# benedikthoward/ENPH459-Super-Resolution

Measured on AMD Instinct MI355X. Metric: HR megapixels/sec at x4 upscale (SAA + 80-iteration IBP reconstruction), higher is better.
Workload: dtype f32; 1 GPU; C2: x4 multi-frame SR of 64x64 LR patches -> 256x256 HR, N=16 frames (all 4x4 sub-pixel phases), 7x7 Gaussian PSF, shift_and_add + ibp(80 it, step 0.5); patches_per_gpu=1024, global_patches=1024, factor=4, frames=16, n_iter=80, parallelism=patch-sharded x1, no collective

## Files before the change

### enph459-super-resolution_amd/csrc/srx_patch.hpp

```cpp
#pragma once
#include "srx_mosaic.hpp"

namespace srx {
namespace patch {

#ifndef SRX_PARK16
#define SRX_PARK16 1
#endif
#ifndef SRX_ADDTID
#define SRX_ADDTID 1
#endif
#ifndef SRX_M0_NOP
#define SRX_M0_NOP "s_nop 0\n\t"
#endif
#ifndef SRX_TRANSPOSE_DEF
#define SRX_TRANSPOSE_DEF 1
#endif
#ifndef SRX_PATCH_DBG
#define SRX_PATCH_DBG 0
#endif
constexpr int PN = 256;
constexpr int TSD = 68;
constexpr int RW = 32 * TSD;
constexpr int SLOT0 = 0, SLOT1 = 1024;
constexpr int FIX = 16;
constexpr int YW = 260;
constexpr int OFF_YT = 16 * RW, OFF_YL = OFF_YT + 4 * YW, OFF_GT = OFF_YL + 4 * YW, OFF_GL = OFF_GT + 3 * YW,
              OFF_ROW = OFF_GL + 3 * YW, OFF_PART = OFF_ROW + PN, LDS_WORDS = OFF_PART + 32;
static_assert(LDS_WORDS * 4 <= 160 * 1024, "LDS budget");

constexpr double ZD = -0.26794919243112270647;
constexpr float PZ = (float)ZD;
constexpr float K2 = (float)(1.0 / (1.0 - ZD));
constexpr float K1 = (float)(1.0 / ((1.0 - ZD) * (1.0 - ZD)));
constexpr float K3 = (float)(ZD / (1.0 - ZD * ZD));
constexpr float K4 = (float)(1.0 / (1.0 - ZD * ZD));
struct ZPow {
    float v[FIX];
    constexpr ZPow() : v()
    {
        double p = ZD;
        for (int i = 0; i < FIX; i++) {
            v[i] = (float)p;
            p *= ZD;
        }
    }
};
__device__ constexpr ZPow ZP{};

typedef float f8 __attribute__((ext_vector_type(8)));
struct AxisW {
    float kb[8];
    float kt[8];
    float wfb[8];
};
struct AxisC {
    int ex;
    int nb;
    int E;
};
__device__ __forceinline__ f8 sload8(const float *p)
{
    f8 v;
    asm volatile("s_load_dwordx8 %0, %1, 0x0\n\ts_waitcnt lgkmcnt(0)" : "=s"(v) : "s"(p) : "memory");
    return v;
}

constexpr int NN_PAD = 2048;

struct PatchArgs {
    AxisC y, x;
    int nn, ntop;
    int ngrp;
    int c01;
    unsigned long long ry[4], rx[4];
    float sn;
};

struct PatchTabs {
    const float *Mt;
    const unsigned *Mt8;
    const int *m8;
    const float *Ct;
    const AxisW *aw;
    const uint2 *nrec;
    const uint2 *nent;
    const float2 *Mn;
    const float *k2;
};

static inline bool axis_ok(const mosaic::AxisPlan &pl, int f)
{
    const int nmin = pl.nmin, nmax = pl.nmax;
    return !pl.zero && nmax >= 0 && nmax <= 1 && nmin <= 0 && nmax - nmin <= 3 && nmax - nmin <= f - 1 && -nmin < f;
}

static inline bool shape_admits(int elem_bytes, int H, int W) { return elem_bytes == 4 && H == PN && W == PN; }

static inline bool eligible(int elem_bytes, int N, int H, int W, const double *sh, const double *k, int kh, int kw, int f, bool rank1_only = false)
{
    if (!shape_admits(elem_bytes, H, W) || f < 2)
        return false;
    mosaic::AxisPlan py, px;
    if (!mosaic::plan_axis(N, sh, 0, f, py) || !mosaic::plan_axis(N, sh, 1, f, px))
        return false;
    fused::Kernel7<float> kc;
    fused::make_kernel7<float>(k, kh, kw, false, kc);
    if (!((kc.separable || !rank1_only) && axis_ok(py, f) && axis_ok(px, f)))
        return false;
    const int exy = py.nmax, nby = -py.nmin, exx = px.nmax, nbx = -px.nmin;
    return (exy + nby) * (PN + exx) + (PN - nby) * (exx + nbx) <= NN_PAD;
}

__global__ void __launch_bounds__(256)
    k_patch_prep(const float *__restrict__ Mg, const float *__restrict__ Cg, int B, int Hg, int Wg, int nby, int nbx, float *__restrict__ Mt,
                 float *__restrict__ Ct, unsigned *__restrict__ Mt8, int *__restrict__ m8)
{
    __shared__ float t[32][33];
    const int b = blockIdx.z, x0 = blockIdx.x * 32, y0 = blockIdx.y * 32;
    const float *src = b < B ? Mg + (size_t)b * Hg * Wg : Cg;
    float *dst = b < B ? Mt + (size_t)b * PN * PN : Ct;
    bool ok = true;
    for (int r = threadIdx.y; r < 32; r += 8) {
        float v = src[(size_t)(y0 + r + 13) * Wg + x0 + threadIdx.x + 13];
        if (b < B && (y0 + r < nby || x0 + (int)threadIdx.x < nbx))
            v = 0.f;
        ok = ok && v == rintf(v) && v >= 0.f && v <= 255.f;
        t[r][threadIdx.x] = v;
    }
    __syncthreads();
    const int g = threadIdx.y;
    reinterpret_cast<float4 *>(dst)[(size_t)(x0 / 4 + g) * PN + y0 + threadIdx.x] =
        make_float4(t[threadIdx.x][4 * g], t[threadIdx.x][4 * g + 1], t[threadIdx.x][4 * g + 2], t[threadIdx.x][4 * g + 3]);
    if (b < B) {
        const unsigned w = (unsigned)t[threadIdx.x][4 * g] | (unsigned)t[threadIdx.x][4 * g + 1] << 8 |
                           (unsigned)t[threadIdx.x][4 * g + 2] << 16 | (unsigned)t[threadIdx.x][4 * g + 3] << 24;
        const int wr = x0 / 4 + g;
        Mt8[(size_t)b * (PN / 4) * PN + ((size_t)(wr >> 2) * PN + y0 + threadIdx.x) * 4 + (wr & 3)] = w;
    }
    const bool bad = __syncthreads_or(b < B && !ok);
    if (bad && threadIdx.x == 0 && threadIdx.y == 0)
        atomicAnd(&m8[b], 0);
}

__device__ __forceinline__ void near_coords(int t, int exy, int exx, int nby, int nbx, int &ngy, int &ngx, int &dst)
{
    const int WN = PN + exx, LN = exx + nbx, ntop = (exy + nby) * WN;
    if (t < ntop) {
        const int rr = t / WN, cc = t - rr * WN;
        ngy = rr - exy, ngx = cc - exx, dst = rr * YW + cc;
    } else {
        const int q = t - ntop, rr = q / LN, cc = q - rr * LN;
        ngy = nby + rr, ngx = cc - exx, dst = 3 * YW + rr * 3 + cc;
    }
}
__device__ __forceinline__ int strip_off(int ry, int rx, int exy, int exx, int nby)
{
    return ry <= nby ? (ry + exy) * YW + rx + exx : 4 * YW + (ry + exy) * 4 + rx + exx;
}

__global__ void __launch_bounds__(256)
    k_patch_near_tab(const int *__restrict__ ncu, const int *__restrict__ nyx, int NS, int PBy, int PBx, int exy, int exx, int nby,
                     int nbx, int Ey, int Ex, int nn, uint2 *__restrict__ nrec, uint2 *__restrict__ nent)
{
    const int t = blockIdx.x * 256 + threadIdx.x;
    if (t >= nn)
        return;
    int ngy, ngx, dst;
    near_coords(t, exy, exx, nby, nbx, ngy, ngx, dst);
    const int ni = mosaic::near_index(ngy + 13, ngx + 13, PN + 27, PBy, PBx), pk = ncu[ni], cnt = pk & 255, cu = pk >> 8;
    const int own = strip_off(ngy, ngx, exy, exx, nby);
    nrec[t] = make_uint2((unsigned)cnt | (unsigned)cu << 8 | (unsigned)dst << 16, (unsigned)own);
    for (int g = 0; g < NS / 4; g++) {
        unsigned o[4];
        for (int e = 0; e < 4; e++) {
            const int c = nyx[(size_t)ni * NS + 4 * g + e];
            o[e] = 4 * g + e < cnt ? (unsigned)strip_off((c & 0xffff) - Ey, (c >> 16) - Ex, exy, exx, nby) : (unsigned)own;
        }
        nent[(size_t)g * NN_PAD + t] = make_uint2(o[0] | o[1] << 16, o[2] | o[3] << 16);
    }
}

__global__ void __launch_bounds__(256)
    k_patch_near_m(const float *__restrict__ Mg, const float *__restrict__ Mu, int NB, int PBy, int PBx, int exy, int exx, int nby, int nbx,
                   int nn, float2 *__restrict__ Mn)
{
    const int t = blockIdx.x * 256 + threadIdx.x, b = blockIdx.y;
    if (t >= nn)
        return;
    int ngy, ngx, dst;
    near_coords(t, exy, exx, nby, nbx, ngy, ngx, dst);
    const int Wg = PN + 27, ni = mosaic::near_index(ngy + 13, ngx + 13, Wg, PBy, PBx);
    Mn[(size_t)b * NN_PAD + t] = make_float2(Mg[((size_t)b * Wg + ngy + 13) * Wg + ngx + 13], Mu[(size_t)b * NB + ni]);
}

struct AxisMap {
    signed char cls[PN];
    unsigned char idx[PN];
};
struct BuildMaps {
    AxisMap y, x;
    signed char frame[4][4];
    int nby, nbx;
};
__global__ void k_patch_maps(BuildMaps v, BuildMaps *dst)
{
    const int *s = reinterpret_cast<const int *>(&v);
    int *d = reinterpret_cast<int *>(dst);
    for (int i = threadIdx.x; i < (int)(sizeof(BuildMaps) / 4); i += blockDim.x)
        d[i] = s[i];
}
template <int PASS, typename S = float, bool WIDE = false>
__global__ void __launch_bounds__(256)
    k_patch_build(const S *__restrict__ lr, int N, int h, int w, const BuildMaps *__restrict__ maps, int *__restrict__ m8,
                  float *__restrict__ Mt, unsigned *__restrict__ Mt8)
{
    __shared__ float4 tile[64][17];
    const int b = blockIdx.y, gy0 = blockIdx.x * 16, cq = threadIdx.x & 63, wv = threadIdx.x >> 6;
    constexpr bool bytes = PASS == 0, test = PASS == 0 && std::is_same<S, float>::value;
    static_assert(PASS == 0 || std::is_same<S, float>::value, "byte frames need no float plane");
    if (PASS == 1 && __builtin_amdgcn_readfirstlane(m8[b]) != 0)
        return;
    int bad = 0;
    const S *src = lr + (size_t)b * N * h * w;
    int cx[4], jx[4];
#pragma unroll
    for (int c = 0; c < 4; c++) {
        const int gx = 4 * cq + c;
        cx[c] = gx < maps->nbx ? -1 : maps->x.cls[gx];
        jx[c] = maps->x.idx[gx];
    }
    const int *fw = reinterpret_cast<const int *>(&maps->frame[0][0]);
    const int fr0 = fw[0], fr1 = fw[1], fr2 = fw[2], fr3 = fw[3];
    float v[4][4];
    bool done = false;
    if constexpr (WIDE) {
        __shared__ unsigned rowsw[4][4][64];
        if ((((size_t)lr) & 3) == 0) {
            const int nd = w >> 2, kx = cq / nd, dw = cq - kx * nd;
            unsigned wd[4];
#pragma unroll
            for (int m = 0; m < 4; m++) {
                const int gy = gy0 + wv + 4 * m;
                const int cy = gy < maps->nby ? -1 : (int)maps->y.cls[gy], iy = maps->y.idx[gy];
                const int fsel = cy == 0 ? fr0 : cy == 1 ? fr1 : cy == 2 ? fr2 : fr3;
                wd[m] = 0;
                if (cy >= 0)
                    wd[m] = reinterpret_cast<const unsigned *>(src + ((size_t)((fsel >> (8 * kx)) & 0xff) * h + iy) * w)[dw];
            }
#pragma unroll
            for (int m = 0; m < 4; m++)
                rowsw[wv][m][cq] = wd[m];
            __syncthreads();
            const unsigned char *rb = reinterpret_cast<const unsigned char *>(&rowsw[wv][0][0]);
#pragma unroll
            for (int m = 0; m < 4; m++) {
                const int gy = gy0 + wv + 4 * m;
                const int cy = gy < maps->nby ? -1 : (int)maps->y.cls[gy];
#pragma unroll
                for (int c = 0; c < 4; c++) {
                    v[m][c] = 0.f;
                    if (cy >= 0 && cx[c] >= 0)
                        v[m][c] = (float)rb[m * 256 + cx[c] * w + jx[c]];
                }
            }
            done = true;
        }
    }
    if (!done)
#pragma unroll
    for (int m = 0; m < 4; m++) {
        const int gy = gy0 + wv + 4 * m;
        const int cy = gy < maps->nby ? -1 : (int)maps->y.cls[gy], iy = maps->y.idx[gy];
        const int fsel = cy == 0 ? fr0 : cy == 1 ? fr1 : cy == 2 ? fr2 : fr3;
#pragma unroll
        for (int c = 0; c < 4; c++) {
            v[m][c] = 0.f;
            if (cy >= 0 && cx[c] >= 0)
                v[m][c] = src[((size_t)((fsel >> (8 * cx[c])) & 0xff) * h + iy) * w + jx[c]];
        }
    }
#pragma unroll
    for (int m = 0; m < 4; m++) {
        if (test) {
#pragma unroll
            for (int c = 0; c < 4; c++)
                bad |= !((int)(v[m][c] == rintf(v[m][c])) & (int)(v[m][c] >= 0.f) & (int)(v[m][c] <= 255.f));
        }
        tile[cq][wv + 4 * m] = make_float4(v[m][0], v[m][1], v[m][2], v[m][3]);
    }
    if (test) {
        if (__syncthreads_or(bad) && threadIdx.x == 0)
            atomicAnd(&m8[b], 0);
    } else {
        __syncthreads();
    }
    if (bytes) {
#pragma unroll
        for (int n = 0; n < 4; n++) {
            const int u = threadIdx.x + 256 * n, sub = u & 3, r = (u >> 2) & 15, grp = u >> 6, q = 4 * grp + sub;
            const float4 t = tile[q][r];
            const unsigned wd = (unsigned)t.x | (unsigned)t.y << 8 | (unsigned)t.z << 16 | (unsigned)t.w << 24;
            Mt8[(size_t)b * (PN / 4) * PN + ((size_t)grp * PN + gy0 + r) * 4 + sub] = wd;
        }
    } else {
#pragma unroll
        for (int n = 0; n < 4; n++) {
            const int u = threadIdx.x + 256 * n, r = u & 15, q = u >> 4;
            reinterpret_cast<float4 *>(Mt)[((size_t)b * (PN / 4) + q) * PN + gy0 + r] = tile[q][r];
        }
// ... 178 lines not shown
        for (int i = 0; i < FIX; i++)
            a[i] = fmaf(ZP.v[i], carry, a[i]);
    }
    const float cb = last ? fmaf(a[63] - blast * K2, K3, blast * K1) : 0.f;
    chain64<true>(a, cb);
    float cm1 = 0.f, cm2 = 0.f;
    if (first) {
        const float qs = bfirst * K2;
        cm1 = fmaf(z, a[0], qs);
        cm2 = fmaf(z, cm1, qs);
        const float cm3 = fmaf(z, cm2, qs);
        yex = wfb[0] * cm3 + wfb[1] * cm2 + wfb[2] * cm1 + wfb[3] * a[0];
    }
    Rown[sb + lane] = a[0];
    Rown[sb + 64 + lane] = a[62];
    Rown[sb + 128 + lane] = a[63];
    __syncthreads();
    float hb = cb;
    if (!last) {
        hb = Rnext[sb + lane];
#pragma unroll
        for (int i = 0; i < FIX; i++)
            a[63 - i] = fmaf(ZP.v[i], hb, a[63 - i]);
    }
    if (!first) {
        cm2 = fmaf(ZP.v[1], a[0], Rprev[sb + 64 + lane]);
        cm1 = fmaf(ZP.v[0], a[0], Rprev[sb + 128 + lane]);
    }
    float c2 = cm2, c1 = cm1;
#pragma unroll
    for (int i = 0; i < 64; i++) {
        const float c0 = a[i], cn = i < 63 ? a[i + 1] : hb;
        a[i] = wfb[0] * c2 + wfb[1] * c1 + wfb[2] * c0 + wfb[3] * cn;
        c2 = c1, c1 = c0;
    }
}

template <bool BLUR, typename F, typename P>
__device__ __forceinline__ void bwd_chain_x(float (&a)[64], float (&out)[64], bool first, bool last, float *Rown, const float *Rprev,
                                            const float *Rnext, int s1, int s6, int lane, const f8 wfb, const f8 kt, float gm1, float gp1,
                                            float gp2, float gtop, F mid, P post, float (&hlo)[3], float (&hhi)[3])
{
    const float z = PZ;
    const float w0 = wfb[4], w1 = wfb[5], w2 = wfb[6], w3 = wfb[7];
    const float vn = last ? w0 * a[63] : 0.f;
    SRX_PSTAMP(15);
    float st = 0.f;
    if (first) {
        st = (w0 + w1 + w2 + w3) * gtop * K2;
        st = fmaf(z, st, (w0 + w1 + w2) * gtop + w3 * a[0]);
        st = fmaf(z, st, (w0 + w1) * gtop + w2 * a[0] + w3 * a[1]);
    }
    float gprev = gm1;
#pragma unroll
    for (int t = 0; t < 64; t++) {
        const float g0 = a[t], g1 = t < 63 ? a[t + 1] : gp1, g2 = t < 62 ? a[t + 2] : (t == 62 ? gp1 : gp2);
        a[t] = w0 * gprev + w1 * g0 + w2 * g1 + w3 * g2;
        gprev = g0;
    }
    chain64<false>(a, st);
    SRX_PSTAMP(16);
    Rown[s1 + lane] = a[63];
    __syncthreads();
    SRX_PSTAMP(17);
    if (!first) {
        const float carry = Rprev[s1 + lane];
#pragma unroll
        for (int i = 0; i < FIX; i++)
            a[i] = fmaf(ZP.v[i], carry, a[i]);
    }
    const float cb = last ? fmaf(z, a[63], vn) * K4 : 0.f;
    chain64<true>(a, cb);
    Rown[s6 + lane] = a[0];
    Rown[s6 + 64 + lane] = a[1];
    Rown[s6 + 128 + lane] = a[2];
    Rown[s6 + 192 + lane] = a[61];
    Rown[s6 + 256 + lane] = a[62];
    Rown[s6 + 320 + lane] = a[63];
    SRX_PSTAMP(18);
    __syncthreads();
    SRX_PSTAMP(19);
    float e[70];
    e[0] = e[1] = e[2] = e[67] = e[68] = e[69] = 0.f;
    if (!last) {
        const float cn = Rnext[s6 + lane];
#pragma unroll
        for (int i = 0; i < FIX; i++)
            a[63 - i] = fmaf(ZP.v[i], cn, a[63 - i]);
        e[67] = cn, e[68] = Rnext[s6 + 64 + lane], e[69] = Rnext[s6 + 128 + lane];
    }
    if (!first) {
        e[0] = fmaf(ZP.v[2], a[0], Rprev[s6 + 192 + lane]);
        e[1] = fmaf(ZP.v[1], a[0], Rprev[s6 + 256 + lane]);
        e[2] = fmaf(ZP.v[0], a[0], Rprev[s6 + 320 + lane]);
    }
#pragma unroll
    for (int i = 0; i < 64; i++)
        e[3 + i] = a[i];
    SRX_PSTAMP(20);
    if (!BLUR) {
        hlo[0] = e[0], hlo[1] = e[1], hlo[2] = e[2], hhi[0] = e[67], hhi[1] = e[68], hhi[2] = e[69];
#pragma unroll
        for (int i = 0; i < 64; i++)
            out[i] = e[3 + i];
        return;
    }
#pragma unroll
    for (int q = 0; q < 4; q++) {
        mid(q);
#pragma unroll
        for (int i = 16 * q; i < 16 * q + 16; i++) {
            float acc = kt[0] * e[i];
#pragma unroll
            for (int u = 1; u < 7; u++)
                acc = fmaf(kt[u], e[i + u], acc);
            out[i] = post(i, acc);
        }
        __builtin_amdgcn_sched_barrier(0);
    }
}

template <typename F, typename P>
__device__ __forceinline__ void bwd_chain(float (&a)[64], float (&out)[64], bool first, bool last, float *Rown, const float *Rprev,
                                          const float *Rnext, int s1, int s6, int lane, const f8 wfb, const f8 kt, float gm1, float gp1,
                                          float gp2, float gtop, F mid, P post)
{
    float hlo[3], hhi[3];
    bwd_chain_x<true>(a, out, first, last, Rown, Rprev, Rnext, s1, s6, lane, wfb, kt, gm1, gp1, gp2, gtop, mid, post, hlo, hhi);
}

__device__ __forceinline__ void blur_block(float (&a)[64], bool first, bool last, float *Rown, const float *Rprev, const float *Rnext,
                                           int s6, int lane, const f8 kb)
{
    Rown[s6 + lane] = a[0];
    Rown[s6 + 64 + lane] = a[1];
    Rown[s6 + 128 + lane] = a[2];
    Rown[s6 + 192 + lane] = a[61];
    Rown[s6 + 256 + lane] = a[62];
    Rown[s6 + 320 + lane] = a[63];
    __syncthreads();
    float hl[3] = {0.f, 0.f, 0.f}, hr[3] = {0.f, 0.f, 0.f};
    if (!first)
        hl[0] = Rprev[s6 + 192 + lane], hl[1] = Rprev[s6 + 256 + lane], hl[2] = Rprev[s6 + 320 + lane];
    if (!last)
        hr[0] = Rnext[s6 + lane], hr[1] = Rnext[s6 + 64 + lane], hr[2] = Rnext[s6 + 128 + lane];
    float c0 = hl[0], c1 = hl[1], c2 = hl[2];
#pragma unroll
    for (int j0 = 0; j0 < 64; j0 += 8) {
        float w[14];
        w[0] = c0, w[1] = c1, w[2] = c2;
#pragma unroll
        for (int j = 0; j < 8; j++)
            w[3 + j] = a[j0 + j];
#pragma unroll
        for (int j = 0; j < 3; j++)
            w[11 + j] = j0 + 8 + j < 64 ? a[j0 + 8 + j] : hr[j];
        c0 = w[8], c1 = w[9], c2 = w[10];
#pragma unroll
        for (int j = 0; j < 8; j++) {
            float acc = kb[0] * w[j];
#pragma unroll
            for (int k = 1; k < 7; k++)
                acc = fmaf(kb[k], w[j + k], acc);
            a[j0 + j] = acc;
        }
        __builtin_amdgcn_sched_barrier(0);
    }
}

typedef float f2 __attribute__((ext_vector_type(2)));
typedef float f4 __attribute__((ext_vector_type(4)));
__device__ __forceinline__ float lane_up(float v) { return __int_as_float(__builtin_amdgcn_update_dpp(0, __float_as_int(v), 0x138, 0xf, 0xf, true)); }
__device__ __forceinline__ float lane_dn(float v) { return __int_as_float(__builtin_amdgcn_update_dpp(0, __float_as_int(v), 0x130, 0xf, 0xf, true)); }
constexpr int SLOT_E = 1536;
constexpr int SLOT_D = 512;
constexpr int SLOT_Z = 2048;
static_assert(SLOT_D >= SLOT0 + 448 && SLOT_D + 256 <= SLOT1 && SLOT_E >= SLOT1 + 448 && SLOT_E + 512 <= SLOT_Z && SLOT_Z + 8 <= RW, "slots inside the wave's region");

#ifndef SRX_PATCH_B2D_NB
#define SRX_PATCH_B2D_NB 4
#endif
template <int RAD>
__device__ __forceinline__ void blur2d_pass1(float (&a)[64], const float (&hl)[3], const float (&hr)[3], float *Rown, int lane, const float *w56)
{
    static_assert(RAD == 2 || RAD == 3, "5 x 5 core or full 7 x 7");
    constexpr int LO = 3 - RAD, HI = 3 + RAD;
    f8 kw[7];
#pragma unroll
    for (int c = 0; c < 7; c++)
        kw[c] = sload8(w56 + 8 * c);
    if (lane < 8)
        Rown[SLOT_Z + lane] = 0.f;
    f4 *edst = reinterpret_cast<f4 *>(__builtin_assume_aligned(lane == 63 ? Rown + SLOT_E : lane == 0 ? Rown + SLOT_E + 4 : Rown + SLOT_D + 4 * lane, 16));
    const int estr = (lane == 63 || lane == 0) ? 2 : 0;
    constexpr int NB = SRX_PATCH_B2D_NB;
    float c0 = hl[0], c1 = hl[1], c2 = hl[2];
#pragma unroll
    for (int j0 = 0; j0 < 64; j0 += NB) {
        float w[NB + 6];
        w[0] = c0, w[1] = c1, w[2] = c2;
#pragma unroll
        for (int j = 0; j < NB; j++)
            w[3 + j] = a[j0 + j];
#pragma unroll
        for (int j = 0; j < 3; j++)
            w[NB + 3 + j] = j0 + NB + j < 64 ? a[j0 + NB + j] : hr[j];
        c0 = w[NB], c1 = w[NB + 1], c2 = w[NB + 2];
#pragma unroll
        for (int j = 0; j < NB; j++) {
            float t[7];
#pragma unroll
            for (int c = LO; c <= HI; c++) {
                t[c] = kw[c][LO] * w[j + LO];
#pragma unroll
                for (int r = LO + 1; r <= HI; r++)
                    t[c] = fmaf(kw[c][r], w[j + r], t[c]);
            }
            float u1, u2, u3, d1, d2, d3;
            if (RAD == 3) {
                u1 = t[0], d1 = t[6];
                u2 = t[1] + lane_up(u1), d2 = t[5] + lane_dn(d1);
            } else {
                u1 = 0.f, d1 = 0.f;
                u2 = t[1], d2 = t[5];
            }
            u3 = t[2] + lane_up(u2), d3 = t[4] + lane_dn(d2);
            const float res = (t[3] + lane_up(u3)) + lane_dn(d3);
            const f4 ev = lane == 0 ? (f4){d1, d2, d3, 0.f} : (f4){u1, u2, u3, 0.f};
            edst[(j0 + j) * estr] = ev;
            a[j0 + j] = res;
            asm volatile("" : "+v"(a[j0 + j]));
        }
        __builtin_amdgcn_sched_barrier(0);
    }
}
template <int RAD, typename PRE, typename POST>
__device__ __forceinline__ void blur2d_fix(float (&a)[64], bool lfirst, bool llast, float *Rown, const float *Rlo, const float *Rhi, int lane, PRE pre, POST post)
{
    const float *src = lane < 3 ? (lfirst ? Rown + SLOT_Z : Rlo + SLOT_E + 2 - lane) : lane >= 61 ? (llast ? Rown + SLOT_Z : Rhi + SLOT_E + 4 + lane - 61) : Rown + SLOT_Z;
    const int str = (lane < 3 ? !lfirst : lane >= 61 ? !llast : false) ? 8 : 0;
#pragma unroll
    for (int q = 0; q < 4; q++) {
        pre(q);
#pragma unroll
        for (int i = 16 * q; i < 16 * q + 16; i++)
            a[i] = post(i, a[i] + src[i * str]);
        __builtin_amdgcn_sched_barrier(0);
    }
}

struct AxisWPair {
    AxisW y, x;
};
struct K2Pair {
    float v[112];
};
__global__ void k_patch_k2(K2Pair t, float *__restrict__ dst)
{
    if (threadIdx.x < 112)
        dst[threadIdx.x] = t.v[threadIdx.x];
}
__global__ void k_patch_params(AxisWPair v, AxisW *dst)
{
    dst[0] = v.y;
    dst[1] = v.x;
}

template <bool C01, bool M8, int PSF = 0>
__global__ void __launch_bounds__(1024)
    k_ibp_patch(const float *__restrict__ hr_in, float *__restrict__ hr_out, PatchTabs tb, PatchArgs pa, const double *__restrict__ Vtot,
                double scale, double *__restrict__ errors, int n_iter)
{
    __shared__ __attribute__((aligned(16))) float lds[LDS_WORDS];
    const int tid0 = threadIdx.x;
    const int wave = __builtin_amdgcn_readfirstlane(tid0 >> 6), s = wave >> 2, u = wave & 3;
    const int b = blockIdx.x;
    float *Rown = lds + wave * RW;
    const float *Rup = lds + (wave - 4) * RW, *Rdn = lds + (wave + 4) * RW;
    const float *Rlf = lds + (wave - 1) * RW, *Rrt = lds + (wave + 1) * RW;
    float *Ystrip = lds + OFF_YT, *Gstrip = lds + OFF_GT, *rowbuf = lds + OFF_ROW;
    float *Yt = lds + OFF_YT, *Yl = lds + OFF_YL, *Gt = lds + OFF_GT, *Gl = lds + OFF_GL;
    double *part = reinterpret_cast<double *>(lds + OFF_PART);
    const int exy = pa.y.ex, exx = pa.x.ex, nby = pa.y.nb, nbx = pa.x.nb;

    const __amdgpu_buffer_rsrc_t rs_in = fused::plane_rsrc(hr_in + (size_t)b * PN * PN, (size_t)PN * PN);
    const __amdgpu_buffer_rsrc_t rs_out = fused::plane_rsrc(hr_out + (size_t)b * PN * PN, (size_t)PN * PN);
    if ((__builtin_amdgcn_readfirstlane(tb.m8[b]) != 0) != M8)
        return;
    constexpr int m8 = M8 ? 1 : 0;
    const float *awy = tb.aw[0].kb, *awx = tb.aw[1].kb;
    const int nn = pa.nn;
    const float sn = pa.sn;
    const int cb0 = (64 * s * PN + 64 * u) * 4;
    const int tb0 = (16 * u * PN + 64 * s) * 16;
    const unsigned long long rmask = C01 ? pa.ry[s] : 0ull, cmask = C01 ? pa.rx[u] : 0ull;

    float a[64];
    {
        const int l4 = (tid0 & 63) * 4;
#pragma unroll
        for (int i = 0; i < 64; i++)
            a[i] = fused::buf_load<float>(rs_in, l4 + (i & 3) * PN * 4, cb0 + (i >> 2) * PN * 16);
    }
#if SRX_PARK16
    asm volatile("s_waitcnt vmcnt(0)" ::: "memory");
    __syncthreads();
    const int park0 = wave * 16384;
#endif
    for (int it = 0; it < n_iter; it++) {
        float r[64];
#define SRX_STAGE_LOCALS()                                 \
    int tid = tid0;                                        \
    asm volatile("" : "+v"(tid));                          \
    const int lane = tid & 63, l4 = lane * 4;              \
    int cbl = cb0, tbl = tb0, m8l = (4 * u * PN + 64 * s) * 16; \
    asm volatile("" : "+s"(cbl), "+s"(tbl), "+s"(m8l));    \
    (void)tbl, (void)m8l, (void)cbl, (void)l4
        float yex = 0.f;
        {
        SRX_STAGE_LOCALS();
        __builtin_amdgcn_sched_barrier(0);
        SRX_PSTAMP(0);
        if (!(SRX_PATCH_DBG & 8)) {
#if SRX_PARK16
            int pk = park0;
            asm volatile("" : "+s"(pk));
#pragma unroll
            for (int q = 0; q < 16; q++)
                st4(rs_out, l4 * 4, pk + q * 1024, a[4 * q], a[4 * q + 1], a[4 * q + 2], a[4 * q + 3]);
#else
#pragma unroll
            for (int i = 0; i < 64; i++)
                fused::buf_store<float>(a[i], rs_out, l4 + (i & 3) * PN * 4, cbl + (i >> 2) * PN * 16);
#endif
        }
        if (PSF == 0) {
            blur_block(a, s == 0, s == 3, Rown, Rup, Rdn, SLOT0, lane, sload8(awy));
        } else {
            Rown[SLOT0 + lane] = a[0];
            Rown[SLOT0 + 64 + lane] = a[1];
            Rown[SLOT0 + 128 + lane] = a[2];
            Rown[SLOT0 + 192 + lane] = a[61];
            Rown[SLOT0 + 256 + lane] = a[62];
            Rown[SLOT0 + 320 + lane] = a[63];
            __syncthreads();
            float hl[3] = {0.f, 0.f, 0.f}, hr[3] = {0.f, 0.f, 0.f};
            if (s != 0)
                hl[0] = Rup[SLOT0 + 192 + lane], hl[1] = Rup[SLOT0 + 256 + lane], hl[2] = Rup[SLOT0 + 320 + lane];
            if (s != 3)
                hr[0] = Rdn[SLOT0 + lane], hr[1] = Rdn[SLOT0 + 64 + lane], hr[2] = Rdn[SLOT0 + 128 + lane];
            blur2d_pass1<PSF == 2 ? 2 : 3>(a, hl, hr, Rown, lane, tb.k2);
            __syncthreads();
            blur2d_fix<PSF == 2 ? 2 : 3>(a, u == 0, u == 3, Rown, Rlf, Rrt, lane, [](int) {}, [](int, float v) { return v; });
#ifdef SRX_PATCH_B2D_SYNC
            __syncthreads();
#endif
        }
        __builtin_amdgcn_sched_barrier(0);
        SRX_PSTAMP(1);
        fwd_chain(a, s == 0, s == 3, Rown, Rup, Rdn, SLOT1, SLOT0, lane, sload8(awy + 16), yex);
        __builtin_amdgcn_sched_barrier(0);
        SRX_PSTAMP(2);
        if (exy && s == 0)
            rowbuf[64 * u + lane] = yex;
        __syncthreads();
        if (exy && s == 3)
            a[63] = rowbuf[64 * u + lane];
        __builtin_amdgcn_sched_barrier(0);
        SRX_PSTAMP(3);
        transpose64(a, r, Rown, lane);
        __builtin_amdgcn_sched_barrier(0);
        SRX_PSTAMP(4);
        }
        float sq = 0.f;
        {
        SRX_STAGE_LOCALS();
        const bool wrapped = exy && s == 3 && lane == 63;
        const int gy = wrapped ? -1 : 64 * s + lane;
        const bool rownear = wrapped || gy < nby;
        const float crow = C01 ? (float)((rmask >> lane) & 1ull) : 0.f;
        if (PSF == 0)
            blur_block(r, u == 0, u == 3, Rown, Rlf, Rrt, SLOT0, lane, sload8(awx));
        __builtin_amdgcn_sched_barrier(0);
        __builtin_amdgcn_sched_barrier(0);
        SRX_PSTAMP(5);
        float yexx = 0.f;
        fwd_chain(r, u == 0, u == 3, Rown, Rlf, Rrt, SLOT1, SLOT0, lane, sload8(awx + 16), yexx);
        __builtin_amdgcn_sched_barrier(0);
        SRX_PSTAMP(6);
        uint2 nr0 = make_uint2(0, 0), nr1 = make_uint2(0, 0), ne0 = make_uint2(0, 0), ne1 = make_uint2(0, 0);
        float2 nm0 = make_float2(0.f, 0.f), nm1 = make_float2(0.f, 0.f);
        const bool n0 = tid < nn, n1 = tid + 1024 < nn;
        const __amdgpu_buffer_rsrc_t rsNr = fused::plane_rsrc(tb.nrec, (size_t)nn), rsNe = fused::plane_rsrc(tb.nent, (size_t)pa.ngrp * NN_PAD),
                                     rsMn = fused::plane_rsrc(tb.Mn + (size_t)b * NN_PAD, (size_t)nn);
        {
            const int t8 = tid * 8;
            nr0 = ld_u2(rsNr, t8), ne0 = ld_u2(rsNe, t8);
            nr1 = ld_u2(rsNr, t8 + 8192), ne1 = ld_u2(rsNe, t8 + 8192);
            const uint2 m0 = ld_u2(rsMn, t8), m1 = ld_u2(rsMn, t8 + 8192);
            nm0 = make_float2(__uint_as_float(m0.x), __uint_as_float(m0.y)), nm1 = make_float2(__uint_as_float(m1.x), __uint_as_float(m1.y));
        }
        {
            const bool toprow = wrapped || (s == 0 && lane <= nby);
            if (toprow) {
                float *dst = Yt + (gy + exy) * YW + 64 * u + exx;
#pragma unroll
                for (int j = 0; j < 64; j++)
                    dst[j] = r[j];
                if (u == 0 && exx)
                    dst[-1] = yexx;
            }
            if (u == 0) {
                float *dst = Yl + (gy + exy) * 4 + exx;
#pragma unroll
                for (int j = 0; j < 3; j++)
                    if (j <= nbx)
                        dst[j] = r[j];
                if (exx)
                    dst[-1] = yexx;
            }
        }
        __syncthreads();
        const __amdgpu_buffer_rsrc_t rsM8 = fused::plane_rsrc(tb.Mt8 + (size_t)b * (PN / 4) * PN, (size_t)(PN / 4) * PN);
        unsigned m8w[16];
        if (m8) {
#pragma unroll
            for (int q = 0; q < 4; q++) {
                const u32x4 v = (SRX_PATCH_DBG & 1) ? u32x4{0x01020304u, 0x01020304u, 0x01020304u, 0x01020304u}
                                                    : __builtin_amdgcn_raw_buffer_load_b128(rsM8, l4 * 4, m8l + q * PN * 16, 0);
                m8w[4 * q] = v.x, m8w[4 * q + 1] = v.y, m8w[4 * q + 2] = v.z, m8w[4 * q + 3] = v.w;
            }
        }
        __builtin_amdgcn_sched_barrier(0);
        SRX_PSTAMP(7);
        {
            auto near_px = [&](uint2 nr, uint2 ne, float2 nm, int t) {
                const int cnt = nr.x & 255, cu = (nr.x >> 8) & 255, dst = nr.x >> 16;
                float ys = (cnt > 0 ? Ystrip[ne.x & 0xffff] : 0.f) + (cnt > 1 ? Ystrip[ne.x >> 16] : 0.f) +
                           (cnt > 2 ? Ystrip[ne.y & 0xffff] : 0.f) + (cnt > 3 ? Ystrip[ne.y >> 16] : 0.f);
                for (int g = 1; 4 * g < cnt; g++) {
                    const uint2 e = ld_u2(rsNe, (g * NN_PAD + t) * 8);
                    const int c = cnt - 4 * g;
                    ys += (c > 0 ? Ystrip[e.x & 0xffff] : 0.f) + (c > 1 ? Ystrip[e.x >> 16] : 0.f) + (c > 2 ? Ystrip[e.y & 0xffff] : 0.f) +
                          (c > 3 ? Ystrip[e.y >> 16] : 0.f);
                }
                Gstrip[dst] = nm.x - ys;
                if (cu > 0) {
                    const float gu = nm.y - (float)cu * Ystrip[nr.y];
                    sq += (SRX_PATCH_DBG & 64) ? 0.f : gu * gu / (float)cu;
                }
            };
            if (n0 && !(SRX_PATCH_DBG & 4))
                near_px(nr0, ne0, nm0, tid);
            if (n1 && !(SRX_PATCH_DBG & 4))
                near_px(nr1, ne1, nm1, tid + 1024);
        }
        __syncthreads();
        __builtin_amdgcn_sched_barrier(0);
        SRX_PSTAMP(8);
        float gexx = 0.f;
        {
            const __amdgpu_buffer_rsrc_t rsM = fused::plane_rsrc(tb.Mt + (size_t)b * PN * PN, (size_t)PN * PN);
            const __amdgpu_buffer_rsrc_t rsC = fused::plane_rsrc(tb.Ct, (size_t)PN * PN);
            float sqf = 0.f;
            unsigned long long cm = cmask;
            asm volatile("" : "+s"(cm));
            float gn[3] = {0.f, 0.f, 0.f};
            if (m8) {
                float cq[4] = {0.f, 0.f, 0.f, 0.f};
#pragma unroll
                for (int j = 0; j < 64; j++) {
                    const float mv = (float)((m8w[j >> 2] >> (8 * (j & 3))) & 255u);
                    float g, w;
                    if (C01) {
                        const bool on = (cm >> j) & 1ull;
                        g = on ? fmaf(-crow, r[j], mv) : 0.f;
                        w = 1.f;
                    } else {
                        if ((j & 3) == 0)
                            ld4(rsC, l4 * 4, tbl + (j >> 2) * PN * 16, cq[0], cq[1], cq[2], cq[3]);
                        const float cv = cq[j & 3];
                        g = fmaf(-cv, r[j], mv);
                        w = mosaic::rcp_count(cv);
                    }
                    const float g2 = g * g * w;
                    sqf += g2;
                    if (j < 3)
                        gn[j] = g2;
                    r[j] = g;
                }
            } else {
#pragma unroll
                for (int j0 = 0; j0 < 64; j0 += 16) {
                    float mv[16], cv[16];
#pragma unroll
                    for (int q = 0; q < 4; q++) {
                        ld4(rsM, l4 * 4, tbl + ((j0 >> 2) + q) * PN * 16, mv[4 * q], mv[4 * q + 1], mv[4 * q + 2], mv[4 * q + 3]);
                        if (C01) {
#pragma unroll
                            for (int c = 0; c < 4; c++)
                                cv[4 * q + c] = ((cm >> (j0 + 4 * q + c)) & 1ull) ? crow : 0.f;
                        } else {
                            ld4(rsC, l4 * 4, tbl + ((j0 >> 2) + q) * PN * 16, cv[4 * q], cv[4 * q + 1], cv[4 * q + 2], cv[4 * q + 3]);
                        }
                    }
#pragma unroll
                    for (int j = 0; j < 16; j++) {
                        const float g = fmaf(-cv[j], r[j0 + j], mv[j]);
                        const float g2 = g * g * (C01 ? 1.f : mosaic::rcp_count(cv[j]));
                        sqf += g2;
                        if (j0 + j < 3)
                            gn[j0 + j] = g2;
                        r[j0 + j] = g;
                    }
                }
            }
            if (u == 0)
                sqf -= (nbx > 0 ? gn[0] : 0.f) + (nbx > 1 ? gn[1] : 0.f) + (nbx > 2 ? gn[2] : 0.f);
            sq += (rownear || (SRX_PATCH_DBG & 32)) ? 0.f : sqf;
            if (rownear) {
                const float *src = Gt + (gy + exy) * YW + 64 * u + exx;
#pragma unroll
                for (int j = 0; j < 64; j++)
                    r[j] = src[j];
                if (u == 0 && exx)
                    gexx = src[-1];
            } else if (u == 0) {
                const float *src = Gl + (gy - nby) * 3 + exx;
#pragma unroll
                for (int j = 0; j < 3; j++)
                    if (j < nbx)
                        r[j] = src[j];
                if (exx)
                    gexx = src[-1];
            }
        }
        if (errors) {
            const double ws = wave_sum((double)sq);
            if (lane == 0)
                part[wave] = ws;
        }
        __builtin_amdgcn_sched_barrier(0);
        SRX_PSTAMP(9);
        {
            Rown[SLOT1 + lane] = r[0];
            Rown[SLOT1 + 64 + lane] = r[1];
            Rown[SLOT1 + 128 + lane] = r[63];
            __syncthreads();
            if (errors && tid == 0) {
                double t = 0.0;
#pragma unroll
                for (int i = 0; i < 16; i++)
                    t += part[i];
                errors[(size_t)b * n_iter + it] = (t + Vtot[b]) * scale;
            }
            const float gtop = exx ? gexx : r[0];
            const float gm1 = u == 0 ? gtop : Rlf[SLOT1 + 128 + lane];
            const float gp1 = u == 3 ? 0.f : Rrt[SLOT1 + lane], gp2 = u == 3 ? 0.f : Rrt[SLOT1 + 64 + lane];
            float hlo[3], hhi[3];
            bwd_chain_x<PSF == 0>(r, a, u == 0, u == 3, Rown, Rlf, Rrt, SLOT0 + 384, SLOT0, lane, sload8(awx + 16), sload8(awx + 8), gm1, gp1, gp2, gtop, [](int) {},
                                  [](int, float v) { return v; }, hlo, hhi);
        }
        __builtin_amdgcn_sched_barrier(0);
        SRX_PSTAMP(10);
        __syncthreads();
        __builtin_amdgcn_sched_barrier(0);
        SRX_PSTAMP(11);
        transpose64(a, r, Rown, lane);
        __builtin_amdgcn_sched_barrier(0);
        SRX_PSTAMP(12);
        }
        {
        SRX_STAGE_LOCALS();
        float hv[16], hw[16];
        {
            if (exy && s == 3) {
                rowbuf[64 * u + lane] = r[63];
                r[63] = 0.f;
            }
            Rown[SLOT0 + lane] = r[0];
            Rown[SLOT0 + 64 + lane] = r[1];
            Rown[SLOT0 + 128 + lane] = r[63];
            __syncthreads();
            const float gtop = exy ? rowbuf[64 * u + lane] : r[0];
            const float gm1 = s == 0 ? gtop : Rup[SLOT0 + 128 + lane];
            const float gp1 = s == 3 ? 0.f : Rdn[SLOT0 + lane], gp2 = s == 3 ? 0.f : Rdn[SLOT0 + 64 + lane];
            auto mid = [&](int q) {
                          auto load16 = [&](float(&ld)[16], int bq) {
#if SRX_PARK16
                              int pk = park0;
                              asm volatile("" : "+s"(pk));
#pragma unroll
                              for (int q = 0; q < 4; q++) {
                                  if (SRX_PATCH_DBG & 2)
                                      ld[4 * q] = ld[4 * q + 1] = ld[4 * q + 2] = ld[4 * q + 3] = 1.f;
                                  else
                                      ld4(rs_out, l4 * 4, pk + (4 * bq + q) * 1024, ld[4 * q], ld[4 * q + 1], ld[4 * q + 2], ld[4 * q + 3]);
                              }
#else
#pragma unroll
                              for (int i = 0; i < 16; i++)
                                  ld[i] = (SRX_PATCH_DBG & 2) ? 1.f : fused::buf_load<float>(rs_out, l4 + (i & 3) * PN * 4, cbl + (4 * bq + (i >> 2)) * PN * 16);
#endif
                          };
                          if (q == 0) {
                              SRX_PSTAMP(13);
                              load16(hv, 0), load16(hw, 1);
                          }
                          if (q == 1)
                              load16(hv, 2);
                          else if (q == 2)
                              load16(hw, 3);
                      };
            auto post = [&](int i, float corr) {
                          return __builtin_amdgcn_fmed3f(fmaf(corr, sn, ((i >> 4) & 1) ? hw[i & 15] : hv[i & 15]), 0.f, 255.f);
                      };
            if (PSF == 0) {
                bwd_chain(r, a, s == 0, s == 3, Rown, Rup, Rdn, SLOT1 + 384, SLOT1, lane, sload8(awy + 16), sload8(awy + 8), gm1, gp1, gp2, gtop, mid, post);
            } else {
                float hl[3], hr[3];
                bwd_chain_x<false>(r, a, s == 0, s == 3, Rown, Rup, Rdn, SLOT1 + 384, SLOT1, lane, sload8(awy + 16), sload8(awy + 8), gm1, gp1, gp2, gtop, [](int) {},
                                   [](int, float v) { return v; }, hl, hr);
                blur2d_pass1<PSF == 2 ? 2 : 3>(a, hl, hr, Rown, lane, tb.k2 + 56);
                __syncthreads();
                blur2d_fix<PSF == 2 ? 2 : 3>(a, u == 0, u == 3, Rown, Rlf, Rrt, lane, mid, post);
#ifdef SRX_PATCH_B2D_SYNC
                __syncthreads();
#endif
            }
        }
        __builtin_amdgcn_sched_barrier(0);
        SRX_PSTAMP(14);
        }
#undef SRX_STAGE_LOCALS
    }
    {
#if SRX_PARK16
        asm volatile("s_waitcnt vmcnt(0)" ::: "memory");
        __syncthreads();
#endif
        const int l4 = (tid0 & 63) * 4;
#pragma unroll
        for (int i = 0; i < 64; i++)
            fused::buf_store<float>(a[i], rs_out, l4 + (i & 3) * PN * 4, cb0 + (i >> 2) * PN * 16);
    }
}

static inline void fill_axis(const mosaic::AxisPlan &pl, const float *cfwd, const float *cbwd, AxisC &ax, AxisW &aw)
{
    const double kq = -6.0 * ZD;
    double wv[4];
    fused::host_weights(1.0 - pl.delta, wv);
    for (int i = 0; i < 4; i++)
        aw.wfb[i] = (float)wv[i];
    fused::host_weights(pl.delta, wv);
    for (int i = 0; i < 4; i++)
        aw.wfb[4 + i] = (float)(kq * wv[i]);
    aw.kb[7] = aw.kt[7] = 0.f;
    for (int i = 0; i < 7; i++)
        aw.kb[i] = (float)(kq * (double)cfwd[i]), aw.kt[i] = cbwd[i];
    ax.ex = pl.nmax, ax.nb = -pl.nmin, ax.E = pl.E;
}

static inline bool c01_masks(const mosaic::AxisPlan &py, const mosaic::AxisPlan &px, int N, int f, unsigned long long ry[4],
                             unsigned long long rx[4])
{
    int ny[SRX_MAX_FRAMES], nx[SRX_MAX_FRAMES], cy = 0, cx = 0;
    for (int k = 0; k < N; k++) {
        bool fy = false, fx = false;
        for (int j = 0; j < cy; j++)
            fy = fy || ny[j] == py.n[k];
        for (int j = 0; j < cx; j++)
            fx = fx || nx[j] == px.n[k];
        if (!fy)
            ny[cy++] = py.n[k];
        if (!fx)
            nx[cx++] = px.n[k];
        for (int j = 0; j < k; j++)
            if (py.n[j] == py.n[k] && px.n[j] == px.n[k])
                return false;
    }
    if (cy * cx != N)
        return false;
    for (int i = 0; i < cy; i++)
        for (int j = 0; j < i; j++)
            if ((ny[i] - ny[j]) % f == 0)
                return false;
    for (int i = 0; i < cx; i++)
        for (int j = 0; j < i; j++)
            if ((nx[i] - nx[j]) % f == 0)
                return false;
    for (int w = 0; w < 4; w++)
        ry[w] = rx[w] = 0ull;
    for (int g = 0; g < PN; g++) {
        for (int i = 0; i < cy; i++) {
            const int uu = g + ny[i];
            if (uu >= 0 && uu <= PN - 1 && uu % f == 0)
                ry[g >> 6] |= 1ull << (g & 63);
        }
        for (int i = 0; i < cx; i++) {
            const int uu = g + nx[i];
            if (uu >= 0 && uu <= PN - 1 && uu % f == 0)
                rx[g >> 6] |= 1ull << (g & 63);
        }
    }
    return true;
}

static inline bool axis_map(const mosaic::AxisPlan &pl, int N, int f, AxisMap &am, int cls_of_frame[SRX_MAX_FRAMES], int &ncls)
{
    int nv[SRX_MAX_FRAMES];
    ncls = 0;
    for (int k = 0; k < N; k++) {
        int c = -1;
        for (int j = 0; j < ncls; j++)
            if (nv[j] == pl.n[k])
                c = j;
        if (c < 0) {
            if (ncls == 4)
                return false;
            c = ncls, nv[ncls++] = pl.n[k];
        }
        cls_of_frame[k] = c;
    }
    for (int g = 0; g < PN; g++) {
        am.cls[g] = -1, am.idx[g] = 0;
        for (int c = 0; c < ncls; c++) {
            const int uu = g + nv[c];
            if (uu >= 0 && uu <= PN - 1 && uu % f == 0)
                am.cls[g] = (signed char)c, am.idx[g] = (unsigned char)(uu / f);
        }
    }
    return true;
}

static inline bool builds_itself(const mosaic::AxisPlan &py, const mosaic::AxisPlan &px, int N, int f)
{
    unsigned long long ry[4], rx[4];
    if ((call_flags() & SRX_FLAG_DIAG_NO_ZERO_FUSE) || !c01_masks(py, px, N, f, ry, rx) || PN / f > 255)
        return false;
    BuildMaps bm;
    int cy[SRX_MAX_FRAMES], cx[SRX_MAX_FRAMES], ny, nx;
    return axis_map(py, N, f, bm.y, cy, ny) && axis_map(px, N, f, bm.x, cx, nx) && ny * nx == N;
}

static inline size_t tabs_bytes(int, int B, int N, int, int)
{
    const size_t ngrp = ((size_t)N + 3) / 4;
    return align_up(sizeof(BuildMaps)) + align_up((size_t)B * PN * PN * 4) + align_up((size_t)B * (PN / 4) * PN * 4) + align_up((size_t)B * 4) + align_up((size_t)PN * PN * 4) +
           align_up((size_t)NN_PAD * 8) + align_up(ngrp * NN_PAD * 8) + align_up((size_t)B * NN_PAD * 8) + align_up(2 * sizeof(AxisW)) + align_up(112 * 4);
}

static int upload_k2(const fused::Kernel7<float> &kc, const fused::Kernel7<float> &kt, float *k2, hipStream_t st)
{
    const double kq = -6.0 * ZD;
    K2Pair kv;
    for (int c = 0; c < 7; c++)
        for (int r = 0; r < 8; r++) {
            kv.v[8 * c + r] = r < 7 ? (float)(kq * kq * (double)kc.k[7 * r + c]) : 0.f;
            kv.v[56 + 8 * c + r] = r < 7 ? kt.k[7 * r + c] : 0.f;
        }
    hipLaunchKernelGGL(k_patch_k2, dim3(1), dim3(128), 0, st, kv, k2);
    SRX_CHECK_LAUNCH();
    return SRX_OK;
}

static int iterate(const mosaic::Common<float> &c, const float *hr_init, float *hr, int n_iter, double *errors, Arena &ar, hipStream_t st)
{
    const int B = c.B, N = c.N, f = c.f, NS = c.NS;
    const mosaic::AxisPlan &py = c.py, &px = c.px;
    const int Hg = PN + 27, Wg = PN + 27, ngrp = NS / 4;
    BuildMaps *maps = ar.take<BuildMaps>(1);
    float *Mt = ar.take<float>((size_t)B * PN * PN);
    unsigned *Mt8 = ar.take<unsigned>((size_t)B * (PN / 4) * PN);
    int *m8 = ar.take<int>(B);
    float *Ct = ar.take<float>((size_t)PN * PN);
    uint2 *nrec = ar.take<uint2>(NN_PAD), *nent = ar.take<uint2>((size_t)ngrp * NN_PAD);
    float2 *Mn = ar.take<float2>((size_t)B * NN_PAD);
    AxisW *aw = ar.take<AxisW>(2);
    float *k2 = ar.take<float>(112);
    if (!ar.ok)
        return SRX_E_WORKSPACE;
    PatchArgs pa;
    AxisWPair awp;
    fill_axis(py, c.kc.cy, c.kt.cy, pa.y, awp.y);
    fill_axis(px, c.kc.cx, c.kt.cx, pa.x, awp.x);
    pa.sn = (float)c.step / (float)N;
    pa.ntop = (pa.y.ex + pa.y.nb) * (PN + pa.x.ex);
    pa.nn = pa.ntop + (PN - pa.y.nb) * (pa.x.ex + pa.x.nb);
    pa.ngrp = ngrp;
    if (pa.nn > NN_PAD)
        return SRX_E_UNSUPPORTED;
    pa.c01 = c01_masks(py, px, N, f, pa.ry, pa.rx) ? 1 : 0;
    if (fill_bytes(m8, 0xff, (size_t)B * sizeof(int), st) != hipSuccess)
        return SRX_E_HIP;
    const bool own = c.own_build;
    if (own) {
        BuildMaps bm;
        int cy[SRX_MAX_FRAMES], cx[SRX_MAX_FRAMES], ny, nx;
        axis_map(py, N, f, bm.y, cy, ny);
        axis_map(px, N, f, bm.x, cx, nx);
        for (int a = 0; a < 4; a++)
            for (int b = 0; b < 4; b++)
                bm.frame[a][b] = 0;
        for (int q = 0; q < N; q++)
            bm.frame[cy[q]][cx[q]] = (signed char)q;
        bm.nby = pa.y.nb, bm.nbx = pa.x.nb;
        hipLaunchKernelGGL(k_patch_maps, dim3(1), dim3(256), 0, st, bm, maps);
        SRX_CHECK_LAUNCH();
        if (c.lr_u8) {
            if (!(call_flags() & SRX_FLAG_DIAG_U8_BYTE_LOADS) && c.w % 4 == 0 && nx * c.w <= PN)
                SRX_LAUNCH(KID_PATCH_BUILD, (k_patch_build<0, uint8_t, true>), dim3(PN / 16, B), dim3(256), 0, st, (const uint8_t *)c.lr, N, c.h, c.w, maps, m8, Mt, Mt8);
            else
                SRX_LAUNCH(KID_PATCH_BUILD, (k_patch_build<0, uint8_t>), dim3(PN / 16, B), dim3(256), 0, st, (const uint8_t *)c.lr, N, c.h, c.w, maps, m8, Mt, Mt8);
        } else {
            SRX_LAUNCH(KID_PATCH_BUILD, k_patch_build<0>, dim3(PN / 16, B), dim3(256), 0, st, (const float *)c.lr, N, c.h, c.w, maps, m8, Mt, Mt8);
            SRX_LAUNCH(KID_PATCH_FLAGS, k_patch_build<1>, dim3(PN / 16, B), dim3(256), 0, st, (const float *)c.lr, N, c.h, c.w, maps, m8, Mt, Mt8);
        }
    } else {
        hipLaunchKernelGGL(k_patch_prep, dim3(PN / 32, PN / 32, B + 1), dim3(32, 8), 0, st, c.Mg, c.Cg, B, Hg, Wg, pa.y.nb, pa.x.nb, Mt, Ct, Mt8, m8);
        SRX_CHECK_LAUNCH();
    }
    if (pa.nn > 0) {
        hipLaunchKernelGGL(k_patch_near_tab, dim3(cdiv(pa.nn, 256)), dim3(256), 0, st, c.ncu, c.nyx, NS, py.PB, px.PB, pa.y.ex, pa.x.ex, pa.y.nb,
                           pa.x.nb, pa.y.E, pa.x.E, pa.nn, nrec, nent);
        SRX_CHECK_LAUNCH();
        if (own && c.lr_u8)
            hipLaunchKernelGGL(k_patch_near_build<uint8_t>, dim3(cdiv(pa.nn, 256), B), dim3(256), 0, st, (const uint8_t *)c.lr, N, c.h, c.w, c.tabY, c.tabX, Hg, Wg,
                               py.D, px.D, pa.y.ex, pa.x.ex, pa.y.nb, pa.x.nb, pa.nn, Mn, c.Vtot);
        else if (own)
            hipLaunchKernelGGL(k_patch_near_build<float>, dim3(cdiv(pa.nn, 256), B), dim3(256), 0, st, (const float *)c.lr, N, c.h, c.w, c.tabY, c.tabX, Hg, Wg,
                               py.D, px.D, pa.y.ex, pa.x.ex, pa.y.nb, pa.x.nb, pa.nn, Mn, c.Vtot);
        else
            hipLaunchKernelGGL(k_patch_near_m, dim3(cdiv(pa.nn, 256), B), dim3(256), 0, st, c.Mg, c.Mu, c.NB, py.PB, px.PB, pa.y.ex, pa.x.ex, pa.y.nb,
                               pa.x.nb, pa.nn, Mn);
        SRX_CHECK_LAUNCH();
    }
    hipLaunchKernelGGL(k_patch_params, dim3(1), dim3(1), 0, st, awp, aw);
    SRX_CHECK_LAUNCH();
    const int psf = fused::psf_form(c.kc, c.kt);
    if (psf != 0)
        SRX_TRY(upload_k2(c.kc, c.kt, k2, st));
    PatchTabs tb{Mt, Mt8, m8, Ct, aw, nrec, nent, Mn, k2};
#define SRX_PATCH_PAIR(C01_, PSF_)                                                                                                              \
    do {                                                                                                                                        \
        SRX_LAUNCH(KID_IBP_PATCH, (k_ibp_patch<C01_, true, PSF_>), dim3(B), dim3(1024), 0, st, hr_init, hr, tb, pa, c.Vtot, c.scale, errors, n_iter);  \
        SRX_LAUNCH(KID_IBP_PATCH, (k_ibp_patch<C01_, false, PSF_>), dim3(B), dim3(1024), 0, st, hr_init, hr, tb, pa, c.Vtot, c.scale, errors, n_iter); \
    } while (0)
    if (pa.c01) {
        if (psf == 0)
            SRX_PATCH_PAIR(true, 0);
        else if (psf == 2)
            SRX_PATCH_PAIR(true, 2);
        else
            SRX_PATCH_PAIR(true, 3);
    } else {
        if (psf == 0)
            SRX_PATCH_PAIR(false, 0);
        else if (psf == 2)
            SRX_PATCH_PAIR(false, 2);
        else
            SRX_PATCH_PAIR(false, 3);
    }
#undef SRX_PATCH_PAIR
    return SRX_OK;
}

}
}
```

Measured before the change: 5967 HR-MP/s.

## Stream parked HR update through a windowed load/store loop after backward pass

Moves the per-iteration reload of the parked current estimate out of the backward blur chain's mid/post hooks and into a separate streaming stage after the chain. That stage loads row quads through a sliding window of configurable depth, applies the clamped step update, and stores the result straight back to the park area. This removes the per-iteration park store at the top of each iteration, which now runs only at it==0, and on the last iteration the store is suppressed with a zero-size buffer descriptor. The aim is to cut register pressure inside the chain (hv/hw arrays) and to overlap global loads with the update. The cost is that these loads are no longer hidden behind the blur arithmetic.

```diff
diff --git a/enph459-super-resolution_amd/csrc/srx_patch.hpp b/enph459-super-resolution_amd/csrc/srx_patch.hpp
--- a/enph459-super-resolution_amd/csrc/srx_patch.hpp
+++ b/enph459-super-resolution_amd/csrc/srx_patch.hpp
@@ -4,8 +4,8 @@
 namespace srx {
 namespace patch {
 
-#ifndef SRX_PARK16
-#define SRX_PARK16 1
+#ifndef SRX_PATCH_WIN
+#define SRX_PATCH_WIN 8
 #endif
 #ifndef SRX_ADDTID
 #define SRX_ADDTID 1
@@ -790,11 +790,9 @@
         for (int i = 0; i < 64; i++)
             a[i] = fused::buf_load<float>(rs_in, l4 + (i & 3) * PN * 4, cb0 + (i >> 2) * PN * 16);
     }
-#if SRX_PARK16
     asm volatile("s_waitcnt vmcnt(0)" ::: "memory");
     __syncthreads();
     const int park0 = wave * 16384;
-#endif
     for (int it = 0; it < n_iter; it++) {
         float r[64];
 #define SRX_STAGE_LOCALS()                                 \
@@ -809,18 +807,12 @@
         SRX_STAGE_LOCALS();
         __builtin_amdgcn_sched_barrier(0);
         SRX_PSTAMP(0);
-        if (!(SRX_PATCH_DBG & 8)) {
-#if SRX_PARK16
+        if (it == 0 && !(SRX_PATCH_DBG & 8)) {
             int pk = park0;
             asm volatile("" : "+s"(pk));
 #pragma unroll
             for (int q = 0; q < 16; q++)
                 st4(rs_out, l4 * 4, pk + q * 1024, a[4 * q], a[4 * q + 1], a[4 * q + 2], a[4 * q + 3]);
-#else
-#pragma unroll
-            for (int i = 0; i < 64; i++)
-                fused::buf_store<float>(a[i], rs_out, l4 + (i & 3) * PN * 4, cbl + (i >> 2) * PN * 16);
-#endif
         }
         if (PSF == 0) {
             blur_block(a, s == 0, s == 3, Rown, Rup, Rdn, SLOT0, lane, sload8(awy));
@@ -1060,7 +1052,6 @@
         }
         {
         SRX_STAGE_LOCALS();
-        float hv[16], hw[16];
         {
             if (exy && s == 3) {
                 rowbuf[64 * u + lane] = r[63];
@@ -1074,41 +1065,16 @@
             const float gm1 = s == 0 ? gtop : Rup[SLOT0 + 128 + lane];
             const float gp1 = s == 3 ? 0.f : Rdn[SLOT0 + lane], gp2 = s == 3 ? 0.f : Rdn[SLOT0 + 64 + lane];
             auto mid = [&](int q) {
-                          auto load16 = [&](float(&ld)[16], int bq) {
-#if SRX_PARK16
-                              int pk = park0;
-                              asm volatile("" : "+s"(pk));
-#pragma unroll
-                              for (int q = 0; q < 4; q++) {
-                                  if (SRX_PATCH_DBG & 2)
-                                      ld[4 * q] = ld[4 * q + 1] = ld[4 * q + 2] = ld[4 * q + 3] = 1.f;
-                                  else
-                                      ld4(rs_out, l4 * 4, pk + (4 * bq + q) * 1024, ld[4 * q], ld[4 * q + 1], ld[4 * q + 2], ld[4 * q + 3]);
-                              }
-#else
-#pragma unroll
-                              for (int i = 0; i < 16; i++)
-                                  ld[i] = (SRX_PATCH_DBG & 2) ? 1.f : fused::buf_load<float>(rs_out, l4 + (i & 3) * PN * 4, cbl + (4 * bq + (i >> 2)) * PN * 16);
-#endif
-                          };
-                          if (q == 0) {
+                          if (q == 0)
                               SRX_PSTAMP(13);
-                              load16(hv, 0), load16(hw, 1);
-                          }
-                          if (q == 1)
-                              load16(hv, 2);
-                          else if (q == 2)
-                              load16(hw, 3);
                       };
-            auto post = [&](int i, float corr) {
-                          return __builtin_amdgcn_fmed3f(fmaf(corr, sn, ((i >> 4) & 1) ? hw[i & 15] : hv[i & 15]), 0.f, 255.f);
-                      };
+            auto post = [](int, float v) { return v; };
             if (PSF == 0) {
                 bwd_chain(r, a, s == 0, s == 3, Rown, Rup, Rdn, SLOT1 + 384, SLOT1, lane, sload8(awy + 16), sload8(awy + 8), gm1, gp1, gp2, gtop, mid, post);
             } else {
                 float hl[3], hr[3];
                 bwd_chain_x<false>(r, a, s == 0, s == 3, Rown, Rup, Rdn, SLOT1 + 384, SLOT1, lane, sload8(awy + 16), sload8(awy + 8), gm1, gp1, gp2, gtop, [](int) {},
-                                   [](int, float v) { return v; }, hl, hr);
+                                   post, hl, hr);
                 blur2d_pass1<PSF == 2 ? 2 : 3>(a, hl, hr, Rown, lane, tb.k2 + 56);
                 __syncthreads();
                 blur2d_fix<PSF == 2 ? 2 : 3>(a, u == 0, u == 3, Rown, Rlf, Rrt, lane, mid, post);
@@ -1118,16 +1084,51 @@
             }
         }
         __builtin_amdgcn_sched_barrier(0);
+        SRX_PSTAMP(23);
+        {
+            int pk = park0;
+            asm volatile("" : "+s"(pk));
+            constexpr int WIN = SRX_PATCH_WIN;
+            static_assert(WIN >= 1 && WIN <= 16, "window of the update stream, in row quads");
+            float win[4 * WIN];
+            auto ldq = [&](int q) {
+                           float *w = win + 4 * (q % WIN);
+                           if (SRX_PATCH_DBG & 2)
+                               w[0] = w[1] = w[2] = w[3] = 1.f;
+                           else
+                               ld4(rs_out, l4 * 4, pk + q * 1024, w[0], w[1], w[2], w[3]);
+                       };
+#pragma unroll
+            for (int q = 0; q < WIN; q++)
+                ldq(q);
+#ifdef SRX_STAMPS
+            const bool park = !(SRX_PATCH_DBG & 8);
+#else
+            const bool park = it + 1 < n_iter && !(SRX_PATCH_DBG & 8);
+#endif
+            const __amdgpu_buffer_rsrc_t rs_park = fused::plane_rsrc(hr_out + (size_t)b * PN * PN, park ? (size_t)PN * PN : (size_t)0);
+#pragma unroll
+            for (int q = 0; q < 16; q++) {
+#pragma unroll
+                for (int c = 0; c < 4; c++)
+                    a[4 * q + c] = __builtin_amdgcn_fmed3f(fmaf(a[4 * q + c], sn, win[4 * (q % WIN) + c]), 0.f, 255.f);
+                st4(rs_park, l4 * 4, pk + q * 1024, a[4 * q], a[4 * q + 1], a[4 * q + 2], a[4 * q + 3]);
+                if (q + WIN < 16)
+                    ldq(q + WIN);
+                __builtin_amdgcn_sched_barrier(0);
+            }
+        }
+        __builtin_amdgcn_sched_barrier(0);
         SRX_PSTAMP(14);
         }
 #undef SRX_STAGE_LOCALS
     }
     {
-#if SRX_PARK16
         asm volatile("s_waitcnt vmcnt(0)" ::: "memory");
         __syncthreads();
-#endif
-        const int l4 = (tid0 & 63) * 4;
+        int tid = tid0;
+        asm volatile("" : "+v"(tid));
+        const int l4 = (tid & 63) * 4;
 #pragma unroll
         for (int i = 0; i < 64; i++)
             fused::buf_store<float>(a[i], rs_out, l4 + (i & 3) * PN * 4, cb0 + (i >> 2) * PN * 16);
```

Result: slower. 5852 HR-MP/s (-1.9%).
